# weihaoysgs/ssvio

Hardware: AMD Instinct MI355X
Metric: stereo frames/s (ORB extract + row-band match + triangulate + one local BA per frame) on 1241x376 (higher is better)
Workload: dtype u8 (front-end) + f64 (BA)

## Files before the change

### include/ssx_test_hooks.h

```cpp
#ifndef SSX_TEST_HOOKS_H
#define SSX_TEST_HOOKS_H
#include "ssx.h"

#ifdef __cplusplus
extern "C" {
#endif

SSX_API int32_t ssx_ba_window_selftest(uint32_t seed, int32_t steps);
SSX_API int32_t ssx_ba_window_debug_rewrites(const ssx_ba_window* win);

SSX_API int64_t ssx_debug_kernel_dynamic_lds(const char* kernel);
SSX_API void ssx_debug_set_dense_slabs(int32_t mode);

SSX_API void ssx_debug_set_trial_finish(int32_t mode);

SSX_API double ssx_ba_debug_prepare_seconds(const ssx_ba_problem* prob, int32_t reps);

SSX_API int32_t ssx_ba_debug_upload_format(const ssx_ba_problem* prob);

SSX_API uint64_t ssx_ba_debug_prepare_digest(const ssx_ba_problem* prob, int32_t threads);

typedef struct ssx_orb_plan_info {
  int32_t status, n_buffers;
  uint64_t digest[3];
  uint64_t arena_bytes, buf_off[32], buf_bytes[32];
  int32_t nlevels, out_cap;
  int32_t lvl_rows[8], lvl_cols[8], feat[8], lvl_cell0[9], gauss_tile0[9];
  char error[256];
} ssx_orb_plan_info;
SSX_API ssx_status ssx_orb_debug_plan(int32_t rows, int32_t cols, int32_t images, const ssx_orb_params* prm, int32_t has_mask,
                                      int32_t detect_only, int32_t unchecked, ssx_orb_plan_info* out);


SSX_API ssx_status ssx_ba_linearize(ssx_ctx* ctx, const ssx_ba_problem* prob, double huber_delta, int32_t jac_mode,
                            double* Hpp, double* bp, double* Hll, double* bl, double* Hpl, double* err,
                            double* chi2);

SSX_API ssx_status ssx_orb_stage_level(ssx_ctx* ctx, int32_t image, int32_t level, int32_t blurred,
                                       uint8_t* out, int32_t out_cap, int32_t* rows, int32_t* cols);
SSX_API ssx_status ssx_orb_stage_candidates(ssx_ctx* ctx, int32_t image, int32_t level, int32_t cap,
                                            ssx_keypoint* out, int32_t* n);

SSX_API ssx_status ssx_lk_stage_level(ssx_ctx* ctx, int32_t which, int32_t level, uint8_t* out, int32_t out_cap,
                                      int32_t* rows, int32_t* cols);
SSX_API ssx_status ssx_lk_stage_deriv(ssx_ctx* ctx, int32_t level, int16_t* out, int32_t out_cap, int32_t* rows,
                                      int32_t* cols);

enum { SSX_LK_STAGED = 0, SSX_LK_ARENA = 1, SSX_LK_EACH = 2, SSX_LK_IN_PLACE = 3 };
enum { SSX_LK_K_PYRAMID = 0, SSX_LK_K_PAD_LEVEL0 = 1, SSX_LK_K_PYR_DOWN = 2, SSX_LK_K_SCHARR = 3, SSX_LK_K_TRACK = 4 };
enum { SSX_LK_SPANS = 7, SSX_LK_MAX_LAUNCHES = 32, SSX_LK_MAX_INFO_JOBS = 256 };
typedef struct ssx_lk_call_info {
  int32_t status;
  char error[256];
  int32_t levels, win, pad, rows[8], cols[8], pitch[8];
// ... 50 lines not shown
```

### ssvio_amd/csrc/ctx.hip

```cpp
#include "ctx.hpp"

extern "C" {

int ssx_version(void) { return SSX_VERSION; }

ssx_status ssx_abi_check(int header_version, size_t sizeof_config, size_t sizeof_ba_problem, size_t sizeof_ba_options, size_t sizeof_ba_result,
                         size_t sizeof_window_update)
{
  return (header_version == SSX_VERSION && sizeof_config == sizeof(ssx_config) && sizeof_ba_problem == sizeof(ssx_ba_problem) &&
          sizeof_ba_options == sizeof(ssx_ba_options) && sizeof_ba_result == sizeof(ssx_ba_result) &&
          sizeof_window_update == sizeof(ssx_ba_window_update)) ? SSX_OK : SSX_ERR_UNSUPPORTED;
}

int ssx_device_count(void)
{
  int n = 0;
  if (hipGetDeviceCount(&n) != hipSuccess) return 0;
  return n;
}

ssx_status ssx_ctx_create(const ssx_config* cfg, ssx_ctx** out)
{
  if (!out) return SSX_ERR_INVALID_ARG;
  *out = nullptr;
// ... 8 lines not shown
  if (hipGetDeviceProperties(&prop, dev) == hipSuccess) c->num_cus = prop.multiProcessorCount;
  if (cfg && cfg->cu_count > 0) {
    const int n_cu = c->num_cus > 0 ? c->num_cus : 256;
    if (cfg->cu_first < 0 || cfg->cu_first + cfg->cu_count > n_cu || n_cu > 512) { delete c; return SSX_ERR_INVALID_ARG; }
    c->cu_mask_words = (n_cu + 31) / 32;
    for (int i = cfg->cu_first; i < cfg->cu_first + cfg->cu_count; ++i) c->cu_mask[i >> 5] |= 1u << (i & 31);
  }
  if (cfg && cfg->stream) {
    c->stream = static_cast<hipStream_t>(cfg->stream);
    c->own_stream = false;
  } else {
    if (c->make_stream(&c->stream, false) != hipSuccess) {
      delete c;
      return SSX_ERR_HIP;
    }
    c->own_stream = true;
  }
  (void)hipEventCreate(&c->ev0);
  (void)hipEventCreate(&c->ev1);
  {
    if (c->make_stream(&c->aux, true) != hipSuccess) (void)hipGetLastError();
  }
  (void)hipEventCreateWithFlags(&c->ev_fork, hipEventDisableTiming);
  (void)hipEventCreateWithFlags(&c->ev_join, hipEventDisableTiming);
  (void)hipEventCreateWithFlags(&c->ev_pyr, hipEventDisableTiming);
  (void)hipEventCreateWithFlags(&c->ev_fast0, hipEventDisableTiming);
  *out = c;
  return SSX_OK;
}

void ssx_ctx_destroy(ssx_ctx* ctx)
{
  if (!ctx) return;
  (void)hipSetDevice(ctx->device);
  (void)hipStreamSynchronize(ctx->stream);
  if (ctx->ba && ctx->ba_free) ctx->ba_free(ctx->ba);
  if (ctx->orb && ctx->orb_free) ctx->orb_free(ctx->orb);
  if (ctx->lk && ctx->lk_free) ctx->lk_free(ctx->lk);
  ctx->po_arena.release();
  ctx->po_stage.release();
  ctx->pnp_arena.release();
  ctx->pnp_stage.release();
  if (ctx->ev0) (void)hipEventDestroy(ctx->ev0);
  if (ctx->ev1) (void)hipEventDestroy(ctx->ev1);
  if (ctx->aux) { (void)hipStreamSynchronize(ctx->aux); (void)hipStreamDestroy(ctx->aux); }
  for (int g = 0; g < 3; ++g) {
    if (ctx->grp[g]) { (void)hipStreamSynchronize(ctx->grp[g]); (void)hipStreamDestroy(ctx->grp[g]); }
    if (ctx->grp_ev[g]) (void)hipEventDestroy(ctx->grp_ev[g]);
  }
  if (ctx->ev_fork) (void)hipEventDestroy(ctx->ev_fork);
  if (ctx->ev_join) (void)hipEventDestroy(ctx->ev_join);
  if (ctx->ev_pyr) (void)hipEventDestroy(ctx->ev_pyr);
  if (ctx->ev_fast0) (void)hipEventDestroy(ctx->ev_fast0);
  for (hipEvent_t e : ctx->prof.pool) (void)hipEventDestroy(e);
  if (ctx->own_stream) (void)hipStreamDestroy(ctx->stream);
  delete ctx;
}

const char* ssx_last_error(const ssx_ctx* ctx) { return ctx ? ctx->err : "null ctx"; }

ssx_status ssx_ctx_synchronize(ssx_ctx* ctx)
{
  if (!ctx) return SSX_ERR_INVALID_ARG;
  SSX_HIP_TRY(ctx, hipStreamSynchronize(ctx->stream));
  return SSX_OK;
}

void* ssx_ctx_stream(ssx_ctx* ctx) { return ctx ? static_cast<void*>(ctx->stream) : nullptr; }

void* ssx_host_alloc(size_t bytes)
{
  void* p = nullptr;
  if (bytes == 0 || hipHostMalloc(&p, bytes, hipHostMallocDefault) != hipSuccess) { (void)hipGetLastError(); return nullptr; }
  return p;
}
// ... 42 lines not shown
```

### ssvio_amd/csrc/ctx.hpp

```cpp
#pragma once
#include <hip/hip_runtime.h>

#include <cstdarg>
#include <cstdio>
#include <cstring>
#include <mutex>
#include <string>
#include <vector>

#include "../../include/ssx.h"

#define SSX_PROF(ctx, kid, stmt)                                              \
  do {                                                                        \
    if ((ctx)->prof.on) {                                                     \
      SsxProf::Rec _r{(kid), (ctx)->prof.get(), (ctx)->prof.get()};           \
      (void)hipEventRecord(_r.a, (ctx)->stream);                              \
      stmt;                                                                   \
      (void)hipEventRecord(_r.b, (ctx)->stream);                              \
      (ctx)->prof.recs.push_back(_r);                                         \
    } else {                                                                  \
      stmt;                                                                   \
    }                                                                         \
  } while (0)

// ... 97 lines not shown
  int num_cus = 256;
  uint32_t cu_mask[16] = {0};
  int cu_mask_words = 0;
  hipError_t make_stream(hipStream_t* out, bool low_priority)
  {
    if (cu_mask_words > 0) return hipExtStreamCreateWithCUMask(out, (uint32_t)cu_mask_words, cu_mask);
    if (low_priority) {
      int least = 0, greatest = 0;
      (void)hipDeviceGetStreamPriorityRange(&least, &greatest);
      if (hipStreamCreateWithPriority(out, hipStreamNonBlocking, least) == hipSuccess) return hipSuccess;
      (void)hipGetLastError();
    }
    return hipStreamCreateWithFlags(out, hipStreamNonBlocking);
  }
  char err[512] = {0};
  BaWorkspace* ba = nullptr;
  OrbWorkspace* orb = nullptr;
  void (*ba_free)(BaWorkspace*) = nullptr;
  void (*orb_free)(OrbWorkspace*) = nullptr;
  void* lk = nullptr;
  void (*lk_free)(void*) = nullptr;
  hipEvent_t ev0 = nullptr, ev1 = nullptr;
  hipStream_t aux = nullptr;
  hipEvent_t ev_fork = nullptr, ev_join = nullptr, ev_pyr = nullptr, ev_fast0 = nullptr;
  hipStream_t grp[3] = {nullptr, nullptr, nullptr};
  hipEvent_t grp_ev[3] = {nullptr, nullptr, nullptr};
  int ba_batch_groups = 0;
  SsxProf prof;
  DevBuf po_arena;
  HostBuf po_stage;
  DevBuf pnp_arena;
  HostBuf pnp_stage;
  struct KfBatchStats { int32_t launches = 0, syncs = 0; int64_t bytes_up = 0, bytes_down = 0; } kf_batch;

  std::mutex err_mu;

  void set_error(const char* fmt, ...)
  {
    std::lock_guard<std::mutex> lk(err_mu);
    va_list ap;
    va_start(ap, fmt);
    vsnprintf(err, sizeof(err), fmt, ap);
    va_end(ap);
  }
};
```

### ssvio_amd/csrc/orb.hip

```cpp
#include <algorithm>
#include <cfloat>
#include <cmath>
#include <vector>

#include "ctx.hpp"
#include "kf_batch.hpp"
#include "orb_ws.hpp"
#include "../../include/ssx_test_hooks.h"

namespace ssxorb {

__constant__ __attribute__((aligned(16))) int8_t c_pattern[256 * 4] = {
#include "brief_pattern.inc"
};
__constant__ int c_umax[16] = {15, 15, 15, 15, 14, 14, 14, 13, 13, 12, 11, 10, 9, 8, 6, 3};
__constant__ int c_gauss[7] = {18, 34, 49, 55, 49, 34, 18};
__constant__ int c_ring_dx[16] = {0, 1, 2, 3, 3, 3, 2, 1, 0, -1, -2, -3, -3, -3, -2, -1};
__constant__ int c_ring_dy[16] = {3, 3, 2, 1, 0, -1, -2, -3, -3, -3, -2, -1, 0, 1, 2, 3};

struct ResizeQuad {
  uint32_t s0;
  uint32_t sel0, sel1;
  uint32_t pad;
  uint32_t w[4];
// ... 581 lines not shown

constexpr int OP_NDW = 9;
constexpr int BP = 37, BR = 18;
constexpr int BP_NDW = 10;
constexpr int PATCH_LDS_DW = 31 * OP_NDW + BP * BP_NDW;

struct IcTables { uint2 w[16][8]; };

__device__ __forceinline__ void ic_tables_init(IcTables& tb)
{
  const int t = threadIdx.x;
  if (t < 128) {
    const int av = t >> 3, k = t & 7, dmax = c_umax[av];
    uint32_t w1 = 0, w0 = 0;
#pragma unroll
    for (int j = 0; j < 4; ++j) {
      const int u = 4 * k + j - 15;
      if (u >= -dmax && u <= dmax) { w1 |= (uint32_t)(u + 15) << (8 * j); w0 |= 1u << (8 * j); }
    }
    tb.w[av][k] = make_uint2(w1, w0);
  }
}

__device__ __forceinline__ float ic_angle(const uint32_t* sp, int off, int lane, const IcTables& tb)
{
  int m10 = 0, m01 = 0;
  if (lane < 62) {
    const int row = lane >> 1, half = lane & 1;
    const int v = row - 15, av = v < 0 ? -v : v;
    const uint32_t* rp = sp + row * OP_NDW + 4 * half;
    uint32_t d[5];
#pragma unroll
    for (int k = 0; k < 5; ++k) d[k] = rp[k];
    uint32_t s1 = 0, s0 = 0;
#pragma unroll
    for (int k = 0; k < 4; ++k) {
      const uint32_t px = __builtin_amdgcn_alignbyte(d[k + 1], d[k], off);
      const uint2 w = tb.w[av][4 * half + k];
      s1 = __builtin_amdgcn_udot4(px, w.x, s1, false);
      s0 = __builtin_amdgcn_udot4(px, w.y, s0, false);
    }
    m10 = (int)s1 - 15 * (int)s0;
    m01 = v * (int)s0;
  }
#pragma unroll
  for (int o2 = 32; o2 > 0; o2 >>= 1) { m10 += __shfl_xor(m10, o2); m01 += __shfl_xor(m01, o2); }
  return fast_atan2_deg((float)m01, (float)m10);
}

__device__ __forceinline__ void sincos_deg(float angle_deg, float* c, float* s)
{
  const float factorPI = (float)(3.1415926535897932384626433832795 / 180.f);
  const float ang = angle_deg * factorPI;
// ... 25 lines not shown

__device__ __forceinline__ void brief_pattern_of_lane(int lane, uint32_t pat[4])
{
#pragma unroll
  for (int j = 0; j < 4; ++j) pat[j] = *reinterpret_cast<const uint32_t*>(&c_pattern[(j * 64 + lane) * 4]);
}
__device__ __forceinline__ void brief_words(const uint8_t* sp, int off, float angle, const uint32_t pat[4], unsigned long long words[4])
{
  float a, b;
  sincos_deg(angle, &a, &b);
  const uint8_t* c = sp + BR * (4 * BP_NDW) + BR + off;
#pragma unroll
  for (int j = 0; j < 4; ++j) {
    const int w = (int)pat[j];
    const float x0 = (float)((w << 24) >> 24), y0 = (float)((w << 16) >> 24), x1 = (float)((w << 8) >> 24), y1 = (float)(w >> 24);
    const int r0 = __float2int_rn(x0 * b + y0 * a), c0 = __float2int_rn(x0 * a - y0 * b);
    const int r1 = __float2int_rn(x1 * b + y1 * a), c1 = __float2int_rn(x1 * a - y1 * b);
    const int t0 = c[r0 * (4 * BP_NDW) + c0];
    const int t1 = c[r1 * (4 * BP_NDW) + c1];
    words[j] = __ballot(t0 < t1);
  }
}

constexpr int OB_KPW = 4;
__global__ __launch_bounds__(256) void k_orient_brief(OrbDev o)
{
  __shared__ uint32_t sPatch[4][PATCH_LDS_DW];
  __shared__ IcTables sIc;
  ic_tables_init(sIc);
  __syncthreads();
  const int img = blockIdx.y;
  const int wave = __builtin_amdgcn_readfirstlane(threadIdx.x >> 6), lane = threadIdx.x & 63;
  const int slot0 = (blockIdx.x * 4 + wave) * OB_KPW;
  int cnt[MAX_LEVELS];
#pragma unroll
  for (int l = 0; l < MAX_LEVELS; ++l) cnt[l] = l < o.nlevels ? o.sel_count[img * o.nlevels + l] : 0;
  uint32_t pat[4];
  brief_pattern_of_lane(lane, pat);
  int lvl_of[OB_KPW];
  uint32_t cand[OB_KPW];
  bool ok[OB_KPW];
#pragma unroll
  for (int j = 0; j < OB_KPW; ++j) {
    const int slot = slot0 + j;
    int level = 0, base = 0, n = cnt[0];
#pragma unroll
    for (int l = 1; l < MAX_LEVELS; ++l) {
      const bool next = l < o.nlevels && level == l - 1 && slot >= base + n;
      base = next ? base + n : base;
      level = next ? l : level;
      n = next ? cnt[l] : n;
    }
    const int k = slot - base;
    ok[j] = k < n && slot < o.out_cap;
    if (k < n && slot >= o.out_cap && lane == 0) atomicOr(&o.status[img], 4);
    lvl_of[j] = level;
    cand[j] = ok[j] ? o.sel[(size_t)(img * o.nlevels + level) * SEL_CAP + k] : 0u;
  }
  uint32_t* sp = sPatch[wave];
  const int minB = EDGE_THRESHOLD - 3;
  uint32_t vr[(31 * OP_NDW + 63) / 64], vb[(BP * BP_NDW + 63) / 64];
  int off_o = 0, off_b = 0;
  auto request = [&](int j) {
    const uint32_t p = cand[j];
    const int cx = (int)(p & 0xFFF) + minB, cy = (int)((p >> 12) & 0xFFF) + minB;
    const size_t lvl = (size_t)img * o.pyr_bytes + o.lvl_off[lvl_of[j]];
    const int pitch = o.lvl_pitch[lvl_of[j]];
    off_o = load_patch<31, OP_NDW, 57, 9>(vr, o.pyr + lvl, pitch, cx - 15, cy - 15, lane);
    off_b = load_patch<BP, BP_NDW, 205, 11>(vb, o.blur + lvl, pitch, cx - BR, cy - BR, lane);
  };
  unsigned long long word_prev = 0;
  float angle_prev = 0.f;
  auto store = [&](int j) {
    const int slot = slot0 + j, level = lvl_of[j];
    const uint32_t p = cand[j];
    if (lane < 4) reinterpret_cast<unsigned long long*>(o.out_desc + ((size_t)img * o.out_cap + slot) * 32)[lane] = word_prev;
    if (lane == 0) {
      ssx_keypoint kp;
      const float sc = o.scale[level];
      kp.x = (float)((int)(p & 0xFFF) + minB); kp.y = (float)((int)((p >> 12) & 0xFFF) + minB);
      if (level != 0) { kp.x *= sc; kp.y *= sc; }
      kp.size = (float)(int)(31 * sc);
      kp.angle = angle_prev;
      kp.response = (float)(p >> 24);
      kp.octave = level;
      kp.class_id = -1;
      reinterpret_cast<ssx_keypoint*>(o.out_kps)[(size_t)img * o.out_cap + slot] = kp;
    }
  };
  if (!ok[0]) return;
  request(0);
#pragma unroll
  for (int j = 0; j < OB_KPW; ++j) {
    if (!ok[j]) break;
    const int oo = off_o, ob = off_b;
    write_patch<31, OP_NDW>(sp, vr, lane);
    write_patch<BP, BP_NDW>(sp + 31 * OP_NDW, vb, lane);
    if (j + 1 < OB_KPW && ok[j + 1]) request(j + 1);
    if (j > 0) store(j - 1);
    __builtin_amdgcn_fence(__ATOMIC_RELEASE, "workgroup");
    __builtin_amdgcn_wave_barrier();
    const float angle = ic_angle(sp, oo, lane, sIc);
    unsigned long long words[4];
    brief_words(reinterpret_cast<const uint8_t*>(sp + 31 * OP_NDW), ob, angle, pat, words);
    word_prev = (lane & 2) ? ((lane & 1) ? words[3] : words[2]) : ((lane & 1) ? words[1] : words[0]);
    angle_prev = angle;
    __builtin_amdgcn_wave_barrier();
    if (j + 1 == OB_KPW || !ok[j + 1]) store(j);
  }
}

struct DescribeAt {
  const ssx_keypoint* in;
  ssx_keypoint* out;
  uint8_t* desc;
  uint8_t* keep;
  int n_in;
};

__device__ __forceinline__ void describe_at_wave(const OrbDev& o, const DescribeAt& a, size_t img_off)
{
  __shared__ uint32_t sPatch[4][PATCH_LDS_DW];
  __shared__ IcTables sIc;
  ic_tables_init(sIc);
  const int wave = __builtin_amdgcn_readfirstlane(threadIdx.x >> 6), lane = threadIdx.x & 63;
  const int k = blockIdx.x * 4 + wave;
  bool active = k < a.n_in;
// ... 342 lines not shown

ssx_status plan(ssx_ctx* ctx, int rows, int cols, int I, const ssx_orb_params& prm, bool has_mask, bool detect_only)
{
  OrbWorkspace* ws = get_ws(ctx);
  const PlanKey key{rows, cols, I, detect_only ? 1 : prm.nlevels, prm.nfeatures, prm.ini_th_fast, prm.min_th_fast, has_mask, detect_only, prm.scale_factor};
  char err[PLAN_ERR] = {0};
  ssx_status st = check_key(key, prm, err);
  if (st == SSX_OK && ws->planned && ws->key == key) return SSX_OK;
  OrbPlan p;
  if (st == SSX_OK) st = build_plan(key, p, err);
  if (st != SSX_OK) { ctx->set_error("%s", err); return st; }
  SSX_HIP_TRY(ctx, hipSetDevice(ctx->device));
  SSX_HIP_TRY(ctx, hipStreamSynchronize(ctx->stream));
  SSX_HIP_TRY(ctx, ws->arena.reserve(p.arena_bytes));
  int n = 0;
  for_each_buffer(p, [&](auto*& ptr, size_t) { wire(ptr, ws->arena.as<char>(), p.off[n++]); });
  const OrbDev& d = p.dev;
  if (!p.cells.empty()) SSX_HIP_TRY(ctx, hipMemcpyAsync((void*)d.cells, p.cells.data(), sizeof(Cell) * p.cells.size(), hipMemcpyHostToDevice, ctx->stream));
  if (!p.xtab.empty()) {
    SSX_HIP_TRY(ctx, hipMemcpyAsync((void*)d.rs_xtab, p.xtab.data(), sizeof(ResizeQuad) * p.xtab.size(), hipMemcpyHostToDevice, ctx->stream));
    SSX_HIP_TRY(ctx, hipMemcpyAsync((void*)d.rs_ytab, p.ytab.data(), sizeof(uint2) * p.ytab.size(), hipMemcpyHostToDevice, ctx->stream));
  }
  SSX_HIP_TRY(ctx, hipStreamSynchronize(ctx->stream));
  ws->dev = d; ws->key = key; ws->planned = true;
  return SSX_OK;
}

static int launch_pyramid(ssx_ctx* ctx, const OrbDev& d, hipStream_t s, int images)
{
  int launches = 0;
  for (int l = 1; l < d.nlevels; ++l) {
    if (d.lvl_cols[l] <= 0 || d.lvl_rows[l] <= 0) break;
    const int loops = images > 8 ? RS_LOOP : 1;
    const dim3 grid((d.lvl_cols[l] + 255) / 256, (d.lvl_rows[l] + 4 * RS_ROWS * loops - 1) / (4 * RS_ROWS * loops), images);
    auto kern = d.rs_wide8[l] ? k_resize<true> : k_resize<false>;
    for (int m = 0; m < (d.has_mask ? 2 : 1); ++m) {
      uint8_t* pyr = m ? d.maskpyr : d.pyr;
      SSX_PROF(ctx, KID_ORB_RESIZE, hipLaunchKernelGGL(kern, grid, dim3(64, 4), 0, s, pyr + d.lvl_off[l - 1], pyr + d.lvl_off[l], d.pyr_bytes,
                         d.lvl_pitch[l - 1], d.lvl_rows[l], d.lvl_cols[l], d.lvl_pitch[l], d.rs_xtab + d.rs_xoff[l], d.rs_ytab + d.rs_yoff[l], loops));
      ++launches;
    }
  }
  return launches;
}

ssx_status stage_level0(ssx_ctx* ctx, const uint8_t* imgs_dev, int stride, size_t img_bytes, const uint8_t* masks_dev, int mask_stride, size_t mask_bytes)
{
  OrbWorkspace* ws = get_ws(ctx);
  const OrbDev& d = ws->dev;
  const dim3 grid((d.lvl_cols[0] + 511) / 512, (d.lvl_rows[0] + 3) / 4, d.I);
  SSX_PROF(ctx, KID_ORB_MISC, hipLaunchKernelGGL(k_copy_level0, grid, dim3(64, 4), 0, ctx->stream, imgs_dev, stride, img_bytes, d.pyr, d.pyr_bytes,
                     d.lvl_rows[0], d.lvl_cols[0], d.lvl_pitch[0]));
  if (masks_dev)
    SSX_PROF(ctx, KID_ORB_MISC, hipLaunchKernelGGL(k_copy_level0, grid, dim3(64, 4), 0, ctx->stream, masks_dev, mask_stride, mask_bytes, d.maskpyr,
                       d.pyr_bytes, d.lvl_rows[0], d.lvl_cols[0], d.lvl_pitch[0]));
  SSX_HIP_TRY(ctx, hipGetLastError());
  return SSX_OK;
}

ssx_status run_pipeline(ssx_ctx* ctx)
{
  OrbWorkspace* ws = get_ws(ctx);
  const OrbDev& d = ws->dev;
  hipStream_t s = ctx->stream;
  SSX_HIP_TRY(ctx, hipMemsetAsync(d.status, 0, sizeof(int) * d.I, s));
  constexpr int FAST_WPW = 2;
  if (FAST_WPW * (size_t)d.fast_lds_per_wave > 48 * 1024)
    (void)hipFuncSetAttribute(reinterpret_cast<const void*>(k_fast_cells), hipFuncAttributeMaxDynamicSharedMemorySize,
                              (int)(FAST_WPW * (size_t)d.fast_lds_per_wave));
  auto launch_fast = [&](hipStream_t st, int c0, int c1) {
    if (c1 > c0)
      SSX_PROF_ON(ctx, st, KID_ORB_FAST, hipLaunchKernelGGL(k_fast_cells, dim3((c1 - c0 + FAST_WPW - 1) / FAST_WPW, d.I), dim3(64 * FAST_WPW),
                                                            FAST_WPW * (size_t)d.fast_lds_per_wave, st, d, c0, c1));
  };
  static const bool no_fork_env = getenv("SSX_ORB_NO_FORK") != nullptr;
  const bool fork = !d.detect_only && ctx->aux != nullptr && d.I > 2 && !no_fork_env;
  if (fork) {
    SSX_HIP_TRY(ctx, hipEventRecord(ctx->ev_fork, s));
    SSX_HIP_TRY(ctx, hipStreamWaitEvent(ctx->aux, ctx->ev_fork, 0));
    launch_fast(ctx->aux, 0, d.lvl_cell0[1]);
    SSX_HIP_TRY(ctx, hipEventRecord(ctx->ev_fast0, ctx->aux));
    launch_pyramid(ctx, d, s, d.I);
    SSX_HIP_TRY(ctx, hipEventRecord(ctx->ev_pyr, s));
    SSX_HIP_TRY(ctx, hipStreamWaitEvent(ctx->aux, ctx->ev_pyr, 0));
    SSX_PROF_ON(ctx, ctx->aux, KID_ORB_GAUSS, hipLaunchKernelGGL(k_gauss7, dim3(d.gauss_tile0[d.nlevels], d.I), dim3(256), 0, ctx->aux, d));
    SSX_HIP_TRY(ctx, hipEventRecord(ctx->ev_join, ctx->aux));
    launch_fast(s, d.lvl_cell0[1], d.n_cells);
    SSX_HIP_TRY(ctx, hipStreamWaitEvent(s, ctx->ev_fast0, 0));
  } else {
    launch_pyramid(ctx, d, s, d.I);
    if (!d.detect_only)
      SSX_PROF(ctx, KID_ORB_GAUSS, hipLaunchKernelGGL(k_gauss7, dim3(d.gauss_tile0[d.nlevels], d.I), dim3(256), 0, s, d));
    launch_fast(s, 0, d.n_cells);
  }
  SSX_PROF(ctx, KID_ORB_OCTREE, launch_octree(d, s));
  if (d.detect_only) {
    SSX_PROF(ctx, KID_ORB_MISC, hipLaunchKernelGGL(k_finalize_detect, dim3((SEL_CAP + 255) / 256, d.I), dim3(256), 0, s, d));
  } else {
    const dim3 kgrid((d.out_cap + 4 + 4 * OB_KPW - 1) / (4 * OB_KPW), d.I);
    if (fork) SSX_HIP_TRY(ctx, hipStreamWaitEvent(s, ctx->ev_join, 0));
    SSX_PROF(ctx, KID_ORB_BRIEF, hipLaunchKernelGGL(k_orient_brief, kgrid, dim3(256), 0, s, d));
  }
  SSX_PROF(ctx, KID_ORB_MISC, hipLaunchKernelGGL(k_counts, dim3((d.I + 63) / 64), dim3(64), 0, s, d));
  SSX_HIP_TRY(ctx, hipGetLastError());
  return SSX_OK;
}

namespace {

ssx_status host_image_to_level0(ssx_ctx* ctx, const uint8_t* img, int stride, int rows, int cols, const uint8_t* mask, int mask_stride, size_t up_bytes)
{
  OrbWorkspace* ws = get_ws(ctx);
  const size_t bytes = (size_t)rows * cols;
  uint8_t *hs = ws->stage.as<uint8_t>(), *in = ws->input.as<uint8_t>();
  copy_rows(hs, cols, img, stride, rows, cols);
  if (mask) copy_rows(hs + bytes, cols, mask, mask_stride, rows, cols);
  SSX_HIP_TRY(ctx, hipMemcpyAsync(ws->input.p, hs, up_bytes, hipMemcpyHostToDevice, ctx->stream));
  return stage_level0(ctx, in, cols, bytes, mask ? in + bytes : nullptr, cols, bytes);
}

ssx_status run_host_image(ssx_ctx* ctx, const uint8_t* img, int stride, int rows, int cols, const uint8_t* mask, int mask_stride, const ssx_orb_params& prm, bool detect_only,
                          int cap, ssx_keypoint* kps_out, uint8_t* desc_out, int32_t* n)
{
  ssx_status st = plan(ctx, rows, cols, 1, prm, mask != nullptr, detect_only);
// ... 48 lines not shown
    f(a.out, sizeof(ssx_keypoint) * (size_t)n_in); f(a.desc, (size_t)32 * n_in); f(a.keep, (size_t)n_in);
  };
  const size_t total = carve(nullptr, buffers);
  SSX_HIP_TRY(ctx, ws->input.reserve(total));
  SSX_HIP_TRY(ctx, ws->stage.reserve(total));
  char* base = ws->input.as<char>();
  carve(base, buffers); a.n_in = n_in;
  ssx_keypoint* hk = (ssx_keypoint*)(ws->stage.as<char>() + ((const char*)a.in - base));
  if (levels > 0) {
    for (int i = 0; i < n_kps; ++i)
      for (int l = 0; l < levels; ++l) {
        ssx_keypoint kp = kps[i];
        kp.octave = l; kp.response = -1.f; kp.class_id = i;
        hk[(size_t)i * levels + l] = kp;
      }
  } else if (n_in > 0) {
    memcpy(hk, kps, sizeof(ssx_keypoint) * n_in);
  }
  const size_t up = (const char*)a.out - base;
  st = host_image_to_level0(ctx, img, stride, rows, cols, nullptr, 0, up);
  if (st != SSX_OK) return st;
  hipStream_t s = ctx->stream;
  int launches = 1 + launch_pyramid(ctx, d, s, 1);
  SSX_PROF(ctx, KID_ORB_GAUSS, hipLaunchKernelGGL(k_gauss7, dim3(d.gauss_tile0[d.nlevels], 1), dim3(256), 0, s, d));
  ++launches;
  if (n_in > 0) {
    SSX_PROF(ctx, KID_ORB_BRIEF, hipLaunchKernelGGL(k_describe_at, dim3((n_in + 3) / 4), dim3(256), 0, s, d, a));
    ++launches;
  }
  SSX_HIP_TRY(ctx, hipGetLastError());
  out->base = base; out->total = total; out->kps = a.out; out->desc = a.desc; out->keep = a.keep; out->n_in = n_in;
  out->launches = launches; out->syncs = planned ? 0 : 2; out->bytes_up = up;
  return SSX_OK;
}

ssx_status describe_batch_prepare(ssx_ctx* ctx, int n, const DescribeJob* jobs, int stride, int rows, int cols, const ssx_orb_params& prm, int levels,
                                  bool images_on_device, size_t extra_bytes, DescribedBatch* out)
{
  OrbWorkspace* ws = get_ws(ctx);
  int cap_I = 1;
  while (cap_I < n) cap_I *= 2;
  const PlanKey want{rows, cols, cap_I, prm.nlevels, prm.nfeatures, prm.ini_th_fast, prm.min_th_fast, 0, 0, prm.scale_factor};
  PlanKey have = ws->key;
  have.I = cap_I;
  const bool planned = ws->planned && have == want && ws->key.I >= n;
  if (planned) cap_I = ws->key.I;
  ssx_status st = plan(ctx, rows, cols, cap_I, prm, false, false);
// ... 28 lines not shown
        hk[k0 + (size_t)i * levels + l] = kp;
      }
    k0 += (size_t)q.n_feats * levels;
  }
  out->host_extra = hs; out->dev_extra = base;
  out->kps = okps; out->desc = odesc; out->keep = okeep;
  out->launches = 0; out->syncs = planned ? 0 : 2; out->bytes_up = up;
  out->o_ptr = o_ptr; out->o_in = o_in; out->stride = images_on_device ? stride : cols; out->total = total;
  return SSX_OK;
}

ssx_status describe_batch_launch(ssx_ctx* ctx, int n, const KfJobDev* table, int max_n_in, DescribedBatch* io)
{
  OrbWorkspace* ws = get_ws(ctx);
  OrbDev d = ws->dev;
  d.I = n;
  hipStream_t s = ctx->stream;
  char* base = ws->input.as<char>();
  SSX_HIP_TRY(ctx, hipMemcpyAsync(base, ws->stage.p, io->bytes_up, hipMemcpyHostToDevice, s));
  const dim3 grid((d.lvl_cols[0] + 511) / 512, (d.lvl_rows[0] + 3) / 4, n);
  SSX_PROF(ctx, KID_ORB_MISC, hipLaunchKernelGGL(k_copy_level0_ptrs, grid, dim3(64, 4), 0, s, reinterpret_cast<const uint8_t* const*>(base + io->o_ptr), io->stride,
                                                 d.pyr, d.pyr_bytes, d.lvl_rows[0], d.lvl_cols[0], d.lvl_pitch[0]));
  int launches = 1 + launch_pyramid(ctx, d, s, n);
  SSX_PROF(ctx, KID_ORB_GAUSS, hipLaunchKernelGGL(k_gauss7, dim3(d.gauss_tile0[d.nlevels], n), dim3(256), 0, s, d));
  ++launches;
  DescribeAt a;
  a.in = reinterpret_cast<const ssx_keypoint*>(base + io->o_in);
  a.out = const_cast<ssx_keypoint*>(io->kps); a.desc = const_cast<uint8_t*>(io->desc); a.keep = const_cast<uint8_t*>(io->keep); a.n_in = 0;
  SSX_PROF(ctx, KID_ORB_BRIEF, hipLaunchKernelGGL(k_describe_at_jobs, dim3(std::max((max_n_in + 3) / 4, 1), n), dim3(256), 0, s, d, a, table));
  ++launches;
  SSX_HIP_TRY(ctx, hipGetLastError());
  io->launches = launches;
  return SSX_OK;
}

}

using namespace ssxorb;

extern "C" {

void ssx_orb_default_params(ssx_orb_params* p)
{
  if (!p) return;
  p->nfeatures = 2000; p->scale_factor = 1.2f; p->nlevels = 8; p->ini_th_fast = 20; p->min_th_fast = 7;
}

// ... 187 lines not shown
                              int32_t unchecked, ssx_orb_plan_info* out)
{
  if (!prm || !out) return SSX_ERR_INVALID_ARG;
  *out = ssx_orb_plan_info{};
  const PlanKey key{rows, cols, images, detect_only ? 1 : prm->nlevels, prm->nfeatures, prm->ini_th_fast, prm->min_th_fast, has_mask != 0, detect_only != 0, prm->scale_factor};
  static_assert(sizeof(out->error) == PLAN_ERR, "ssx_orb_plan_info::error holds the plan's error text");
  OrbPlan p;
  ssx_status st = unchecked && key.nlevels >= 1 && key.nlevels <= MAX_LEVELS ? SSX_OK : check_key(key, *prm, out->error);
  if (st == SSX_OK) st = build_plan(key, p, out->error);
  out->status = st;
  if (st != SSX_OK) return st;
  const OrbDev& d = p.dev;
  size_t offs[ARENA_BUFS + 1];
  for (int b = 0; b < ARENA_BUFS; ++b) { out->buf_off[b] = offs[b] = p.off[b]; out->buf_bytes[b] = p.bytes[b]; }
  out->n_buffers = ARENA_BUFS;
  out->arena_bytes = offs[ARENA_BUFS] = p.arena_bytes;
  out->nlevels = d.nlevels; out->out_cap = d.out_cap;
  memcpy(out->lvl_rows, d.lvl_rows, sizeof(d.lvl_rows)); memcpy(out->lvl_cols, d.lvl_cols, sizeof(d.lvl_cols)); memcpy(out->feat, d.feat, sizeof(d.feat));
  memcpy(out->lvl_cell0, d.lvl_cell0, sizeof(d.lvl_cell0)); memcpy(out->gauss_tile0, d.gauss_tile0, sizeof(d.gauss_tile0));
  plan_digest(d, offs, ARENA_BUFS + 1, p.cells, p.xtab, p.ytab, out->digest);
  return SSX_OK;
}

ssx_status ssx_orb_stage_level(ssx_ctx* ctx, int32_t image, int32_t level, int32_t blurred, uint8_t* out,
                               int32_t out_cap, int32_t* rows, int32_t* cols)
{
  if (!ctx || !ctx->orb || !ctx->orb->planned) return SSX_ERR_INVALID_ARG;
  const OrbDev& d = ctx->orb->dev;
  if (image < 0 || image >= d.I || level < 0 || level >= d.nlevels) return SSX_ERR_INVALID_ARG;
  const int r = d.lvl_rows[level], c = d.lvl_cols[level];
  if (rows) *rows = r;
  if (cols) *cols = c;
  if (!out) return SSX_OK;
  if (out_cap < r * c) return SSX_ERR_CAPACITY;
  const uint8_t* src = (blurred ? d.blur : d.pyr) + (size_t)image * d.pyr_bytes + d.lvl_off[level];
  SSX_HIP_TRY(ctx, hipMemcpy2DAsync(out, c, src, d.lvl_pitch[level], c, r, hipMemcpyDeviceToHost, ctx->stream));
  SSX_HIP_TRY(ctx, hipStreamSynchronize(ctx->stream));
  return SSX_OK;
}

ssx_status ssx_orb_stage_candidates(ssx_ctx* ctx, int32_t image, int32_t level, int32_t cap, ssx_keypoint* out,
                                    int32_t* n)
{
  if (!ctx || !ctx->orb || !ctx->orb->planned || !n) return SSX_ERR_INVALID_ARG;
  const OrbDev& d = ctx->orb->dev;
  if (image < 0 || image >= d.I || level < 0 || level >= d.nlevels) return SSX_ERR_INVALID_ARG;
  const int c0 = d.lvl_cell0[level], c1 = d.lvl_cell0[level + 1];
  const int nc = c1 - c0;
  std::vector<int> cnt(std::max(nc, 1));
  std::vector<uint32_t> cand((size_t)std::max(nc, 1) * CELL_CAP);
  if (nc > 0) {
    SSX_HIP_TRY(ctx, hipMemcpyAsync(cnt.data(), d.cell_count + (size_t)image * d.n_cells + c0, sizeof(int) * nc, hipMemcpyDeviceToHost, ctx->stream));
    SSX_HIP_TRY(ctx, hipMemcpyAsync(cand.data(), d.cell_cand + ((size_t)image * d.n_cells + c0) * CELL_CAP,
                                    sizeof(uint32_t) * (size_t)nc * CELL_CAP, hipMemcpyDeviceToHost, ctx->stream));
    SSX_HIP_TRY(ctx, hipStreamSynchronize(ctx->stream));
  }
  int m = 0;
// ... 17 lines not shown
```

### ssvio_amd/csrc/orb_ws.hpp

```cpp
#pragma once
#include <hip/hip_runtime.h>

#include <cstdint>
#include <vector>

#include "ctx.hpp"

namespace ssxorb {

constexpr int MAX_LEVELS = 8;
constexpr int CELL_CAP = 256;
constexpr int CAND_CAP = 16384;
constexpr int CAND_CAP_BIG = 65536;
constexpr int SEL_CAP = 4096;
constexpr int EDGE_THRESHOLD = 19;
constexpr int OCT_THREADS = 1024;

struct Cell {
  int16_t x0, y0;
  int16_t w, h;
  int16_t ox, oy;
  int16_t level, pad;
};

// ... 56 lines not shown
  }
  bool detects_masked(int rows_, int cols_, const ssx_orb_params& prm, int n) const {
    return detect_only && has_mask && rows == rows_ && cols == cols_ && nfeatures == prm.nfeatures && ini_th == prm.ini_th_fast && min_th == prm.min_th_fast && I >= n;
  }
};

struct Ring2 {
  int first = 0, count = 0;
  int push_slot() const { return (first + count) & 1; }
  int pop() { const int s = first; first ^= 1; --count; return s; }
};

void launch_octree(const OrbDev& o, hipStream_t s);

}

struct OrbWorkspace {
  DevBuf arena;
  DevBuf input;
  DevBuf stereo;
  HostBuf stage;
  HostBuf fetch;
  ssxorb::PlanKey key; ssxorb::OrbDev dev{}; bool planned = false;
  const uint8_t* batch_imgs = nullptr;
  int batch_pairs = 0, batch_stride = 0;
  ssx_orb_params batch_orb{};
  ssx_match_params batch_mp{};
  ssx_stereo_rig batch_rig{};
  int *match_idx = nullptr, *match_dist = nullptr, *pair_counts = nullptr;
  double* xyz = nullptr;
  uint8_t* tri_ok = nullptr;
  struct Upload { DevBuf buf; hipEvent_t ev_up = nullptr, ev_free = nullptr; bool free_pending = false; int pairs = 0, stride = 0, rows = 0, cols = 0; } up[2];
  ssxorb::Ring2 up_ring;
  hipStream_t copy_stream = nullptr;
  struct Counts { hipEvent_t ev = nullptr; int pairs = 0; ssx_status fail = SSX_OK; } cnt[2];
  ssxorb::Ring2 cnt_ring;
  HostBuf counts_pinned;
};

namespace ssxorb {
OrbWorkspace* get_ws(ssx_ctx* ctx);
ssx_status plan(ssx_ctx* ctx, int rows, int cols, int I, const ssx_orb_params& prm, bool has_mask, bool detect_only);
ssx_status stage_level0(ssx_ctx* ctx, const uint8_t* imgs_dev, int stride, size_t img_bytes, const uint8_t* masks_dev, int mask_stride, size_t mask_bytes);
ssx_status run_pipeline(ssx_ctx* ctx);
ssx_status fetch_image(ssx_ctx* ctx, int image, int cap, ssx_keypoint* kps_out, uint8_t* desc_out, int32_t* n);
void launch_bf_match(hipStream_t stream, const uint8_t* dq, int nq, const uint8_t* dt, int nt, int* idx, int* dist);
// ... 14 lines not shown
```

Before: 18740.

## Fuse Gaussian blur into orient/BRIEF kernel, dropping separate blur pass

Adds a fused variant of the orientation/BRIEF kernel. It loads a 43x43 raw patch per keypoint, computes the 7-tap Gaussian row sums in LDS with packed dot products, and evaluates the column pass only at the BRIEF sample points. This removes the full-pyramid k_gauss7 launch, its memory traffic, and the aux-stream fork/join events. The cost is extra per-keypoint ALU and LDS work, plus border-reflection handling. The blur buffer is now produced lazily for debug and staging readers, and the old path can still be selected with an env var or a hook.

```diff
diff --git a/include/ssx_test_hooks.h b/include/ssx_test_hooks.h
--- a/include/ssx_test_hooks.h
+++ b/include/ssx_test_hooks.h
@@ -30,6 +30,8 @@
 } ssx_orb_plan_info;
 SSX_API ssx_status ssx_orb_debug_plan(int32_t rows, int32_t cols, int32_t images, const ssx_orb_params* prm, int32_t has_mask,
                                       int32_t detect_only, int32_t unchecked, ssx_orb_plan_info* out);
+
+SSX_API void ssx_orb_debug_set_blur_pass(int32_t mode);
 
 
 SSX_API ssx_status ssx_ba_linearize(ssx_ctx* ctx, const ssx_ba_problem* prob, double huber_delta, int32_t jac_mode,
diff --git a/ssvio_amd/csrc/ctx.hip b/ssvio_amd/csrc/ctx.hip
--- a/ssvio_amd/csrc/ctx.hip
+++ b/ssvio_amd/csrc/ctx.hip
@@ -54,8 +54,6 @@
     if (c->make_stream(&c->aux, true) != hipSuccess) (void)hipGetLastError();
   }
   (void)hipEventCreateWithFlags(&c->ev_fork, hipEventDisableTiming);
-  (void)hipEventCreateWithFlags(&c->ev_join, hipEventDisableTiming);
-  (void)hipEventCreateWithFlags(&c->ev_pyr, hipEventDisableTiming);
   (void)hipEventCreateWithFlags(&c->ev_fast0, hipEventDisableTiming);
   *out = c;
   return SSX_OK;
@@ -81,8 +79,6 @@
     if (ctx->grp_ev[g]) (void)hipEventDestroy(ctx->grp_ev[g]);
   }
   if (ctx->ev_fork) (void)hipEventDestroy(ctx->ev_fork);
-  if (ctx->ev_join) (void)hipEventDestroy(ctx->ev_join);
-  if (ctx->ev_pyr) (void)hipEventDestroy(ctx->ev_pyr);
   if (ctx->ev_fast0) (void)hipEventDestroy(ctx->ev_fast0);
   for (hipEvent_t e : ctx->prof.pool) (void)hipEventDestroy(e);
   if (ctx->own_stream) (void)hipStreamDestroy(ctx->stream);
diff --git a/ssvio_amd/csrc/ctx.hpp b/ssvio_amd/csrc/ctx.hpp
--- a/ssvio_amd/csrc/ctx.hpp
+++ b/ssvio_amd/csrc/ctx.hpp
@@ -143,7 +143,7 @@
   void (*lk_free)(void*) = nullptr;
   hipEvent_t ev0 = nullptr, ev1 = nullptr;
   hipStream_t aux = nullptr;
-  hipEvent_t ev_fork = nullptr, ev_join = nullptr, ev_pyr = nullptr, ev_fast0 = nullptr;
+  hipEvent_t ev_fork = nullptr, ev_fast0 = nullptr;
   hipStream_t grp[3] = {nullptr, nullptr, nullptr};
   hipEvent_t grp_ev[3] = {nullptr, nullptr, nullptr};
   int ba_batch_groups = 0;
diff --git a/ssvio_amd/csrc/orb.hip b/ssvio_amd/csrc/orb.hip
--- a/ssvio_amd/csrc/orb.hip
+++ b/ssvio_amd/csrc/orb.hip
@@ -627,13 +627,14 @@
   }
 }
 
+template <int NDW = OP_NDW>
 __device__ __forceinline__ float ic_angle(const uint32_t* sp, int off, int lane, const IcTables& tb)
 {
   int m10 = 0, m01 = 0;
   if (lane < 62) {
     const int row = lane >> 1, half = lane & 1;
     const int v = row - 15, av = v < 0 ? -v : v;
-    const uint32_t* rp = sp + row * OP_NDW + 4 * half;
+    const uint32_t* rp = sp + row * NDW + 4 * half;
     uint32_t d[5];
 #pragma unroll
     for (int k = 0; k < 5; ++k) d[k] = rp[k];
@@ -705,10 +706,111 @@
   }
 }
 
+constexpr int RP = 43, RR = 21;
+constexpr int RP_NDW = 12;
+constexpr int RS_PITCH = 40;
+constexpr int RS_PAIRS = (RP + 1) / 2;
+constexpr int FUSED_LDS_DW = RP * RP_NDW + RS_PAIRS * RS_PITCH;
+static_assert(BP / 2 + 3 < RS_PAIRS && BP <= RS_PITCH, "the column pass of the last blurred row and column stays inside the row sums");
+static_assert((RP * RP_NDW) % 4 == 0 && FUSED_LDS_DW % 4 == 0, "the row sums are stored as aligned uint4");
+
+__device__ __forceinline__ int load_patch_border(uint32_t (&v)[(RP * RP_NDW + 63) / 64], const uint8_t* src, int pitch, int rows, int cols, int x0, int y0, int lane)
+{
+  const int ax = x0 & ~3, gx_max = (cols - 1) & ~3;
+#pragma unroll
+  for (int i0 = 0; i0 < RP * RP_NDW; i0 += 64) {
+    const int i = i0 + lane;
+    const int r = i / RP_NDW, d = i - r * RP_NDW;
+    int gy = y0 + r;
+    gy = gy < 0 ? -gy : gy;
+    gy = gy >= rows ? 2 * rows - 2 - gy : gy;
+    gy = min(max(gy, 0), rows - 1);
+    const int gx = min(max(ax + 4 * d, 0), gx_max);
+    v[i0 / 64] = i < RP * RP_NDW ? *reinterpret_cast<const uint32_t*>(src + (size_t)gy * pitch + gx) : 0u;
+  }
+  return x0 - ax;
+}
+__device__ __forceinline__ void fused_fix_columns(uint32_t* raw, int cols, int x0, int lane)
+{
+  if (lane < RP) {
+    uint8_t* rb = reinterpret_cast<uint8_t*>(raw + lane * RP_NDW);
+    const int ax = x0 & ~3;
+#pragma unroll
+    for (int k = 0; k < 4; ++k) {
+      const int x = k < 2 ? k - 2 : cols + k - 2;
+      const int xs = k < 2 ? -x : 2 * cols - 2 - x;
+      if (x >= x0 && x < x0 + RP) rb[x - ax] = rb[xs - ax];
+    }
+  }
+}
+constexpr int RS_OCTS = RS_PITCH / 8;
+__device__ __forceinline__ void fused_blur_rows(const uint32_t* raw, uint32_t* sums, int off, int lane)
+{
+  constexpr uint32_t W_LO = 18u | (34u << 8) | (49u << 16) | (55u << 24);
+  constexpr uint32_t W_HI = 49u | (34u << 8) | (18u << 16);
+#pragma unroll 1
+  for (int i0 = 0; i0 < RS_PAIRS * RS_OCTS; i0 += 64) {
+    const int i = i0 + lane;
+    if (i < RS_PAIRS * RS_OCTS) {
+      const int rp = i / RS_OCTS, oc = i - rp * RS_OCTS;
+      uint32_t sum[2][8];
+#pragma unroll
+      for (int h = 0; h < 2; ++h) {
+        const uint32_t* rd = raw + min(2 * rp + h, RP - 1) * RP_NDW + 2 * oc;
+        uint32_t e[4], w[12];
+#pragma unroll
+        for (int k = 0; k < 4; ++k) e[k] = __builtin_amdgcn_alignbyte(rd[k + 1], rd[k], off);
+#pragma unroll
+        for (int j = 0; j < 12; ++j) w[j] = (j & 3) ? __builtin_amdgcn_alignbyte(e[j / 4 + 1], e[j / 4], j & 3) : e[j / 4];
+#pragma unroll
+        for (int j = 0; j < 8; ++j) sum[h][j] = __builtin_amdgcn_udot4(w[j + 4], W_HI, __builtin_amdgcn_udot4(w[j], W_LO, 0u, false), false);
+      }
+      uint32_t pk[8];
+#pragma unroll
+      for (int j = 0; j < 8; ++j) pk[j] = __builtin_amdgcn_perm(sum[1][j], sum[0][j], 0x05040100u);
+      uint4* dst = reinterpret_cast<uint4*>(&sums[rp * RS_PITCH + 8 * oc]);
+      dst[0] = make_uint4(pk[0], pk[1], pk[2], pk[3]);
+      dst[1] = make_uint4(pk[4], pk[5], pk[6], pk[7]);
+    }
+  }
+}
+__device__ __forceinline__ int fused_blur_at(const uint32_t* sums, int r, int c)
+{
+  constexpr uint32_t E0 = 18u | (34u << 16), E1 = 49u | (55u << 16), E2 = 49u | (34u << 16), E3 = 18u;
+  constexpr uint32_t O0 = 18u << 16, O1 = 34u | (49u << 16), O2 = 55u | (49u << 16), O3 = 34u | (18u << 16);
+  const int br = r + BR;
+  const uint32_t* p = sums + (br >> 1) * RS_PITCH + (c + BR);
+  const bool odd = br & 1;
+  uint32_t acc = udot2(p[0], odd ? O0 : E0, 1u << 15);
+  acc = udot2(p[RS_PITCH], odd ? O1 : E1, acc);
+  acc = udot2(p[2 * RS_PITCH], odd ? O2 : E2, acc);
+  acc = udot2(p[3 * RS_PITCH], odd ? O3 : E3, acc);
+  return (int)min(acc >> 16, 255u);
+}
+__device__ __forceinline__ void brief_words_fused(const uint32_t* sums, float angle, const uint32_t pat[4], unsigned long long words[4])
+{
+  float a, b;
+  sincos_deg(angle, &a, &b);
+#pragma unroll
+  for (int j = 0; j < 4; ++j) {
+    const int w = (int)pat[j];
+    const float x0 = (float)((w << 24) >> 24), y0 = (float)((w << 16) >> 24), x1 = (float)((w << 8) >> 24), y1 = (float)(w >> 24);
+    const int r0 = __float2int_rn(x0 * b + y0 * a), c0 = __float2int_rn(x0 * a - y0 * b);
+    const int r1 = __float2int_rn(x1 * b + y1 * a), c1 = __float2int_rn(x1 * a - y1 * b);
+    words[j] = __ballot(fused_blur_at(sums, r0, c0) < fused_blur_at(sums, r1, c1));
+  }
+}
+__device__ __forceinline__ void wave_lds_sync()
+{
+  __builtin_amdgcn_fence(__ATOMIC_RELEASE, "workgroup");
+  __builtin_amdgcn_wave_barrier();
+}
+
 constexpr int OB_KPW = 4;
+template <bool FUSED>
 __global__ __launch_bounds__(256) void k_orient_brief(OrbDev o)
 {
-  __shared__ uint32_t sPatch[4][PATCH_LDS_DW];
+  __shared__ __attribute__((aligned(16))) uint32_t sPatch[4][FUSED ? FUSED_LDS_DW : PATCH_LDS_DW];
   __shared__ IcTables sIc;
   ic_tables_init(sIc);
   __syncthreads();
@@ -742,15 +844,29 @@
   }
   uint32_t* sp = sPatch[wave];
   const int minB = EDGE_THRESHOLD - 3;
-  uint32_t vr[(31 * OP_NDW + 63) / 64], vb[(BP * BP_NDW + 63) / 64];
-  int off_o = 0, off_b = 0;
+  uint32_t vr[((FUSED ? RP * RP_NDW : 31 * OP_NDW) + 63) / 64], vb[FUSED ? 1 : (BP * BP_NDW + 63) / 64];
+  int off_o = 0, off_b = 0, x0_raw = 0, cols_raw = 0;
+  bool fix_cols = false;
   auto request = [&](int j) {
     const uint32_t p = cand[j];
     const int cx = (int)(p & 0xFFF) + minB, cy = (int)((p >> 12) & 0xFFF) + minB;
     const size_t lvl = (size_t)img * o.pyr_bytes + o.lvl_off[lvl_of[j]];
     const int pitch = o.lvl_pitch[lvl_of[j]];
-    off_o = load_patch<31, OP_NDW, 57, 9>(vr, o.pyr + lvl, pitch, cx - 15, cy - 15, lane);
-    off_b = load_patch<BP, BP_NDW, 205, 11>(vb, o.blur + lvl, pitch, cx - BR, cy - BR, lane);
+    if constexpr (FUSED) {
+      const int rows = o.lvl_rows[lvl_of[j]], cols = o.lvl_cols[lvl_of[j]];
+      const int x0 = cx - RR, y0 = cy - RR;
+      x0_raw = x0; cols_raw = cols;
+      fix_cols = x0 < 0 || x0 + RP > cols;
+      int ln = lane;
+      asm volatile("" : "+v"(ln));
+      if (!fix_cols && y0 >= 0 && y0 + RP <= rows && (x0 & ~3) + 4 * RP_NDW <= pitch)
+        off_o = load_patch<RP, RP_NDW, 43, 9>(vr, o.pyr + lvl, pitch, x0, y0, ln);
+      else
+        off_o = load_patch_border(vr, o.pyr + lvl, pitch, rows, cols, x0, y0, ln);
+    } else {
+      off_o = load_patch<31, OP_NDW, 57, 9>(vr, o.pyr + lvl, pitch, cx - 15, cy - 15, lane);
+      off_b = load_patch<BP, BP_NDW, 205, 11>(vb, o.blur + lvl, pitch, cx - BR, cy - BR, lane);
+    }
   };
   unsigned long long word_prev = 0;
   float angle_prev = 0.f;
@@ -777,15 +893,33 @@
   for (int j = 0; j < OB_KPW; ++j) {
     if (!ok[j]) break;
     const int oo = off_o, ob = off_b;
-    write_patch<31, OP_NDW>(sp, vr, lane);
-    write_patch<BP, BP_NDW>(sp + 31 * OP_NDW, vb, lane);
-    if (j + 1 < OB_KPW && ok[j + 1]) request(j + 1);
-    if (j > 0) store(j - 1);
-    __builtin_amdgcn_fence(__ATOMIC_RELEASE, "workgroup");
-    __builtin_amdgcn_wave_barrier();
-    const float angle = ic_angle(sp, oo, lane, sIc);
+    float angle;
     unsigned long long words[4];
-    brief_words(reinterpret_cast<const uint8_t*>(sp + 31 * OP_NDW), ob, angle, pat, words);
+    if constexpr (FUSED) {
+      const bool fix = fix_cols;
+      const int x0 = x0_raw, cols = cols_raw;
+      uint32_t* sums = sp + RP * RP_NDW;
+      write_patch<RP, RP_NDW>(sp, vr, lane);
+      if (j + 1 < OB_KPW && ok[j + 1]) request(j + 1);
+      if (j > 0) store(j - 1);
+      wave_lds_sync();
+      if (fix) {
+        fused_fix_columns(sp, cols, x0, lane);
+        wave_lds_sync();
+      }
+      angle = ic_angle<RP_NDW>(sp + (RR - 15) * RP_NDW + ((oo + RR - 15) >> 2), (oo + RR - 15) & 3, lane, sIc);
+      fused_blur_rows(sp, sums, oo, lane);
+      wave_lds_sync();
+      brief_words_fused(sums, angle, pat, words);
+    } else {
+      write_patch<31, OP_NDW>(sp, vr, lane);
+      write_patch<BP, BP_NDW>(sp + 31 * OP_NDW, vb, lane);
+      if (j + 1 < OB_KPW && ok[j + 1]) request(j + 1);
+      if (j > 0) store(j - 1);
+      wave_lds_sync();
+      angle = ic_angle(sp, oo, lane, sIc);
+      brief_words(reinterpret_cast<const uint8_t*>(sp + 31 * OP_NDW), ob, angle, pat, words);
+    }
     word_prev = (lane & 2) ? ((lane & 1) ? words[3] : words[2]) : ((lane & 1) ? words[1] : words[0]);
     angle_prev = angle;
     __builtin_amdgcn_wave_barrier();
@@ -1174,7 +1308,7 @@
     SSX_HIP_TRY(ctx, hipMemcpyAsync((void*)d.rs_ytab, p.ytab.data(), sizeof(uint2) * p.ytab.size(), hipMemcpyHostToDevice, ctx->stream));
   }
   SSX_HIP_TRY(ctx, hipStreamSynchronize(ctx->stream));
-  ws->dev = d; ws->key = key; ws->planned = true;
+  ws->dev = d; ws->key = key; ws->planned = true; ws->blur_valid = false;
   return SSX_OK;
 }
 
@@ -1208,6 +1342,18 @@
                        d.pyr_bytes, d.lvl_rows[0], d.lvl_cols[0], d.lvl_pitch[0]));
   SSX_HIP_TRY(ctx, hipGetLastError());
   return SSX_OK;
+}
+
+static void launch_gauss(ssx_ctx* ctx, const OrbDev& d, hipStream_t s, int images)
+{
+  SSX_PROF(ctx, KID_ORB_GAUSS, hipLaunchKernelGGL(k_gauss7, dim3(d.gauss_tile0[d.nlevels], images), dim3(256), 0, s, d));
+}
+
+static int g_blur_pass_mode = -1;
+static bool blur_pass_forced()
+{
+  static const bool env = getenv("SSX_ORB_BLUR_PASS") != nullptr;
+  return g_blur_pass_mode < 0 ? env : g_blur_pass_mode != 0;
 }
 
 ssx_status run_pipeline(ssx_ctx* ctx)
@@ -1227,31 +1373,29 @@
   };
   static const bool no_fork_env = getenv("SSX_ORB_NO_FORK") != nullptr;
   const bool fork = !d.detect_only && ctx->aux != nullptr && d.I > 2 && !no_fork_env;
+  const bool blur_pass = !d.detect_only && blur_pass_forced();
   if (fork) {
     SSX_HIP_TRY(ctx, hipEventRecord(ctx->ev_fork, s));
     SSX_HIP_TRY(ctx, hipStreamWaitEvent(ctx->aux, ctx->ev_fork, 0));
     launch_fast(ctx->aux, 0, d.lvl_cell0[1]);
     SSX_HIP_TRY(ctx, hipEventRecord(ctx->ev_fast0, ctx->aux));
     launch_pyramid(ctx, d, s, d.I);
-    SSX_HIP_TRY(ctx, hipEventRecord(ctx->ev_pyr, s));
-    SSX_HIP_TRY(ctx, hipStreamWaitEvent(ctx->aux, ctx->ev_pyr, 0));
-    SSX_PROF_ON(ctx, ctx->aux, KID_ORB_GAUSS, hipLaunchKernelGGL(k_gauss7, dim3(d.gauss_tile0[d.nlevels], d.I), dim3(256), 0, ctx->aux, d));
-    SSX_HIP_TRY(ctx, hipEventRecord(ctx->ev_join, ctx->aux));
+    if (blur_pass) launch_gauss(ctx, d, s, d.I);
     launch_fast(s, d.lvl_cell0[1], d.n_cells);
     SSX_HIP_TRY(ctx, hipStreamWaitEvent(s, ctx->ev_fast0, 0));
   } else {
     launch_pyramid(ctx, d, s, d.I);
-    if (!d.detect_only)
-      SSX_PROF(ctx, KID_ORB_GAUSS, hipLaunchKernelGGL(k_gauss7, dim3(d.gauss_tile0[d.nlevels], d.I), dim3(256), 0, s, d));
+    if (blur_pass) launch_gauss(ctx, d, s, d.I);
     launch_fast(s, 0, d.n_cells);
   }
+  ws->blur_valid = blur_pass;
   SSX_PROF(ctx, KID_ORB_OCTREE, launch_octree(d, s));
   if (d.detect_only) {
     SSX_PROF(ctx, KID_ORB_MISC, hipLaunchKernelGGL(k_finalize_detect, dim3((SEL_CAP + 255) / 256, d.I), dim3(256), 0, s, d));
   } else {
     const dim3 kgrid((d.out_cap + 4 + 4 * OB_KPW - 1) / (4 * OB_KPW), d.I);
-    if (fork) SSX_HIP_TRY(ctx, hipStreamWaitEvent(s, ctx->ev_join, 0));
-    SSX_PROF(ctx, KID_ORB_BRIEF, hipLaunchKernelGGL(k_orient_brief, kgrid, dim3(256), 0, s, d));
+    if (blur_pass) SSX_PROF(ctx, KID_ORB_BRIEF, hipLaunchKernelGGL(k_orient_brief<false>, kgrid, dim3(256), 0, s, d));
+    else SSX_PROF(ctx, KID_ORB_BRIEF, hipLaunchKernelGGL(k_orient_brief<true>, kgrid, dim3(256), 0, s, d));
   }
   SSX_PROF(ctx, KID_ORB_MISC, hipLaunchKernelGGL(k_counts, dim3((d.I + 63) / 64), dim3(64), 0, s, d));
   SSX_HIP_TRY(ctx, hipGetLastError());
@@ -1346,7 +1490,8 @@
   if (st != SSX_OK) return st;
   hipStream_t s = ctx->stream;
   int launches = 1 + launch_pyramid(ctx, d, s, 1);
-  SSX_PROF(ctx, KID_ORB_GAUSS, hipLaunchKernelGGL(k_gauss7, dim3(d.gauss_tile0[d.nlevels], 1), dim3(256), 0, s, d));
+  launch_gauss(ctx, d, s, 1);
+  ws->blur_valid = true;
   ++launches;
   if (n_in > 0) {
     SSX_PROF(ctx, KID_ORB_BRIEF, hipLaunchKernelGGL(k_describe_at, dim3((n_in + 3) / 4), dim3(256), 0, s, d, a));
@@ -1421,7 +1566,8 @@
   SSX_PROF(ctx, KID_ORB_MISC, hipLaunchKernelGGL(k_copy_level0_ptrs, grid, dim3(64, 4), 0, s, reinterpret_cast<const uint8_t* const*>(base + io->o_ptr), io->stride,
                                                  d.pyr, d.pyr_bytes, d.lvl_rows[0], d.lvl_cols[0], d.lvl_pitch[0]));
   int launches = 1 + launch_pyramid(ctx, d, s, n);
-  SSX_PROF(ctx, KID_ORB_GAUSS, hipLaunchKernelGGL(k_gauss7, dim3(d.gauss_tile0[d.nlevels], n), dim3(256), 0, s, d));
+  launch_gauss(ctx, d, s, n);
+  ws->blur_valid = n == ws->dev.I;
   ++launches;
   DescribeAt a;
   a.in = reinterpret_cast<const ssx_keypoint*>(base + io->o_in);
@@ -1655,6 +1801,8 @@
   return SSX_OK;
 }
 
+void ssx_orb_debug_set_blur_pass(int32_t mode) { ssxorb::g_blur_pass_mode = mode; }
+
 ssx_status ssx_orb_stage_level(ssx_ctx* ctx, int32_t image, int32_t level, int32_t blurred, uint8_t* out,
                                int32_t out_cap, int32_t* rows, int32_t* cols)
 {
@@ -1666,6 +1814,11 @@
   if (cols) *cols = c;
   if (!out) return SSX_OK;
   if (out_cap < r * c) return SSX_ERR_CAPACITY;
+  if (blurred && !ctx->orb->blur_valid) {
+    SSX_PROF(ctx, KID_ORB_GAUSS, hipLaunchKernelGGL(k_gauss7, dim3(d.gauss_tile0[d.nlevels], d.I), dim3(256), 0, ctx->stream, d));
+    SSX_HIP_TRY(ctx, hipGetLastError());
+    ctx->orb->blur_valid = true;
+  }
   const uint8_t* src = (blurred ? d.blur : d.pyr) + (size_t)image * d.pyr_bytes + d.lvl_off[level];
   SSX_HIP_TRY(ctx, hipMemcpy2DAsync(out, c, src, d.lvl_pitch[level], c, r, hipMemcpyDeviceToHost, ctx->stream));
   SSX_HIP_TRY(ctx, hipStreamSynchronize(ctx->stream));
diff --git a/ssvio_amd/csrc/orb_ws.hpp b/ssvio_amd/csrc/orb_ws.hpp
--- a/ssvio_amd/csrc/orb_ws.hpp
+++ b/ssvio_amd/csrc/orb_ws.hpp
@@ -102,6 +102,7 @@
   HostBuf stage;
   HostBuf fetch;
   ssxorb::PlanKey key; ssxorb::OrbDev dev{}; bool planned = false;
+  bool blur_valid = false;
   const uint8_t* batch_imgs = nullptr;
   int batch_pairs = 0, batch_stride = 0;
   ssx_orb_params batch_orb{};
```

Result: slower. 18540 (-1.1%).
